# zpelgrims/zoic

Measured on AMD Instinct MI355X. Metric: camera rays/sec (Mrays/s), 4K x 16spp Kolb lens trace; ray-dir RMSE vs CPU ref, higher is better.
Workload: dtype f32

## Files before the change

### zoic_amd/csrc/device_search.hpp

```cpp
#pragma once
#include <hip/hip_runtime.h>

#include "optics.hpp"
#include "tables.hpp"

namespace zoic {

__device__ __forceinline__ int chunk_count_le(const float *chunk, float v)
{
    const float4 *p = reinterpret_cast<const float4 *>(chunk);
    const float4 a = p[0], b = p[1], c = p[2], d = p[3];
    int n = 0;
    n += !(v < a.x); n += !(v < a.y); n += !(v < a.z); n += !(v < a.w);
    n += !(v < b.x); n += !(v < b.y); n += !(v < b.z); n += !(v < b.w);
    n += !(v < c.x); n += !(v < c.y); n += !(v < c.z); n += !(v < c.w);
    n += !(v < d.x); n += !(v < d.y); n += !(v < d.z); n += !(v < d.w);
    return n;
}

__device__ __forceinline__ int pyramid_upper_bound(const float *const level[kBokehMaxLevels], const int32_t stride[kBokehMaxLevels],
                                                   const int32_t count[kBokehMaxLevels], int levels, int row, float v)
{
    int pos = 0;
#pragma unroll
// ... 9 lines not shown
__device__ __forceinline__ V2 bokeh_sample_device(const BokehTables &B, int x, int y, float uRow, float uCol)
{
    if (B.levels == 0)
        return bokeh_sample(B.cdfRow, B.rowIndices, B.cdfColumn, B.columnIndices, x, y, uRow, uCol);
    const int32_t zeroStride[kBokehMaxLevels] = {0, 0, 0};
    int r = pyramid_upper_bound(B.rowLevel, zeroStride, B.rowCount, B.levels, 0, uRow);
    if (r >= y) r = y - 1;
    const int row = B.rowIndices[r];
    int c = pyramid_upper_bound(B.colLevel, B.colStride, B.colCount, B.levels, row, uCol);
    if (c >= x) c = x - 1;
    const int start = row * x;
    const int col = B.columnIndices[start + c] - start;
    const float flippedRow = static_cast<float>(col - ((y - 1) / 2));
    const float flippedColumn = static_cast<float>(row - ((x - 1) / 2)) * -1.0f;
    return V2{(flippedRow / static_cast<float>(x)) * 2.0f, (flippedColumn / static_cast<float>(y)) * 2.0f};
}

__device__ __forceinline__ int cell_of(float u, int cellCount, bool &inRange)
{
    inRange = (u >= 0.0f) & (u < 1.0f);
    return inRange ? static_cast<int>(u * static_cast<float>(cellCount)) : 0;
}

__device__ __forceinline__ int cell_resolve(const uint4 rec, float u, bool inRange, bool &exceptional)
{
    const float a = __builtin_bit_cast(float, rec.x), b = __builtin_bit_cast(float, rec.y);
    const bool ge0 = !(u < a), ge1 = !(u < b);
    exceptional = ((rec.w >> 31) != 0u) | !inRange;
    const uint32_t pair = ge1 ? rec.w : rec.z;
    return static_cast<int>((ge0 & !ge1) ? (pair >> 16) : (pair & 0xffffu));
}

struct CellProbe { uint4 rec; int row; uint32_t cellIndex; };

__device__ __forceinline__ CellProbe bokeh_cells_issue(const BokehTables &B, const float *ldsRowCells, int y, float uRow, float uCol)
{
    bool inR, inC, excR;
    const int gr = cell_of(uRow, B.rowCellCount, inR);
    const int gc = cell_of(uCol, B.colCellCount, inC);
    int row = cell_resolve(reinterpret_cast<const uint4 *>(ldsRowCells)[gr], uRow, inR, excR);
    if (__ballot(excR) != 0ull) {
        if (excR) {
            const uint32_t bnd = B.rowBounds[gr];
            const int lo = inR ? static_cast<int>(bnd & 0xffffu) : 0, hi = inR ? static_cast<int>(bnd >> 16) : y;
            int r = lo + upper_bound_idx(B.cdfRow + lo, hi - lo, uRow);
            if (r >= y) r = y - 1;
            row = B.rowIndices[r];
        }
    }
    CellProbe p;
    p.row = row;
    p.cellIndex = static_cast<uint32_t>(row) * static_cast<uint32_t>(B.colCellCount) + static_cast<uint32_t>(gc);
    p.rec = reinterpret_cast<const uint4 *>(B.colCells)[p.cellIndex];
    return p;
}

template <bool EXACT_DIVIDE>
__device__ __forceinline__ V2 bokeh_cells_finish(const BokehTables &B, int x, int y, float uCol, const CellProbe &p)
{
    const bool inC = (uCol >= 0.0f) & (uCol < 1.0f);
    bool excC;
    const int row = p.row;
    int col = cell_resolve(p.rec, uCol, inC, excC);
    if (__ballot(excC) != 0ull) {
        if (excC) {
            const uint32_t bnd = B.colBounds[p.cellIndex];
            const int lo = inC ? static_cast<int>(bnd & 0xffffu) : 0, hi = inC ? static_cast<int>(bnd >> 16) : x;
            const int start = row * x;
            int c = lo + upper_bound_idx(B.cdfColumn + start + lo, hi - lo, uCol);
            if (c >= x) c = x - 1;
            col = B.columnIndices[start + c] - start;
        }
    }
    const float flippedRow = static_cast<float>(col - ((y - 1) / 2));
    const float flippedColumn = static_cast<float>(row - ((x - 1) / 2)) * -1.0f;
    if constexpr (EXACT_DIVIDE)
        return V2{(flippedRow / static_cast<float>(x)) * 2.0f, (flippedColumn / static_cast<float>(y)) * 2.0f};
    else
        return V2{flippedRow * (2.0f * __builtin_amdgcn_rcpf(static_cast<float>(x))),
                  flippedColumn * (2.0f * __builtin_amdgcn_rcpf(static_cast<float>(y)))};
}

template <bool EXACT_DIVIDE>
__device__ __forceinline__ V2 bokeh_sample_cells(const BokehTables &B, const float *ldsRowCells, int x, int y, float uRow, float uCol)
{
    return bokeh_cells_finish<EXACT_DIVIDE>(B, x, y, uCol, bokeh_cells_issue(B, ldsRowCells, y, uRow, uCol));
}

// ... 2 lines not shown
```

### zoic_amd/csrc/kolb_pool_body.hpp

```cpp
#pragma once
#include <hip/hip_runtime.h>

#include <cstdio>
#include <cstdlib>

#include "kolb_device.hpp"
#include "work_cursor.hpp"

#pragma STDC FP_CONTRACT OFF

#ifndef ZOIC_TWO_LEVEL_SEARCH
#define ZOIC_TWO_LEVEL_SEARCH 3
#endif
constexpr int kTwoLevelDraws = ZOIC_TWO_LEVEL_SEARCH;

namespace zoic {

struct KolbKernelArgs {
    KolbTable T; BokehTables B; const float4 *samples; const uint4 *rngStates; uint64_t rayBase; uint32_t n; RayRecord *out;
    DeviceCounters *counters; unsigned int *workCursor; uint32_t ldsWords, chunkRays, chunksPerPart, minSearching;
    uint32_t *redoList; unsigned int *redoCount;
    unsigned int *clearCursor;
};
template <class V, size_t OFFSET>
__device__ __forceinline__ V kernarg_field()
{
    typedef const char __attribute__((address_space(4))) *KernargBytes;
    KernargBytes base = (KernargBytes)__builtin_amdgcn_kernarg_segment_ptr();
    asm volatile("" : "+s"(base));
    return *(const V __attribute__((address_space(4))) *)(base + OFFSET);
}
#define ZOIC_KARG(field) kernarg_field<decltype(KolbKernelArgs::field), offsetof(KolbKernelArgs, field)>()

constexpr uint32_t kRetryDeadBit = 0x40000000u;

struct RaySetup { float o0x, o0y, maxScale, translation, sn, cs; uint32_t flags; bool dead, lutEdge; uint32_t rminq; };
template <bool STRICT, bool RMIN = false>
__device__ __forceinline__ RaySetup setup_ray(const KolbTable &T, const float2 *lutLds, float sx, float sy)
{
    RaySetup r;
    r.o0x = sx * T.halfSensor;
    r.o0y = sy * T.halfSensor;
    r.maxScale = 0.0f; r.translation = 0.0f; r.sn = 0.0f; r.cs = 1.0f; r.flags = 0u; r.dead = false; r.lutEdge = false; r.rminq = 0u;
    if (T.useLUT) {
        float dist;
// ... 75 lines not shown
    if (states) { const uint4 r = states[idx]; rng = Rng{r.x, r.y, r.z, r.w}; }
    else rng = rng_for_ray(T.seed, rayBase + idx);
    const DeadRayEnd e = dead_ray_end<STRICT>(T, B, bokehLds, rs, rng);
    store_ray_record(out, idx, e.o.x * -1.0f, e.o.y * -1.0f, e.o.z * -1.0f, e.d.x * -1.0f, e.d.y * -1.0f, e.d.z * -1.0f, e.w,
                     1u | (e.tries << 1) | ((rs.flags & 1u) << 6));
    return e.nanDraw;
}

#ifndef ZOIC_SEARCH_DRAWS
#define ZOIC_SEARCH_DRAWS 2
#endif
constexpr uint32_t kPoolEntries = 128;
constexpr uint32_t kPoolWaveWords = kPoolEntries * 12u;
constexpr uint32_t kPoolListWords = 128;
constexpr uint32_t kPoolTriesShift = 8, kPoolDeadBit = 1u << 13, kPoolRetryDeadBit = 1u << 14;

#ifndef ZOIC_POOL_ATTR_FAST
#define ZOIC_POOL_ATTR_FAST __attribute__((amdgpu_waves_per_eu(5, 8)))
#endif
#ifndef ZOIC_POOL_ATTR_STRICT
#define ZOIC_POOL_ATTR_STRICT __attribute__((amdgpu_waves_per_eu(4, 4)))
#endif

__device__ __forceinline__ uint32_t mask_rank(unsigned long long m)
{
    return __builtin_amdgcn_mbcnt_hi(static_cast<uint32_t>(m >> 32), __builtin_amdgcn_mbcnt_lo(static_cast<uint32_t>(m), 0u));
}
__device__ __forceinline__ bool mask_bit(unsigned long long m, uint32_t lane) { return ((m >> lane) & 1ull) != 0ull; }

constexpr uint32_t kShortList = 1u << 17;
template <bool STRICT, int NS, bool GUARD, bool DEAD, bool IMAGE, bool TWO = false>
__device__ __forceinline__ void kolb_pool_body(const KolbTable &T, const BokehTables &B, const float4 *__restrict__ samples,
                                               uint32_t n, RayRecord *__restrict__ out, uint32_t ldsWords, uint32_t minSearching)
{
    static_assert(!(GUARD && STRICT), "GUARD is a FAST mode");
    static_assert(!TWO || (DEAD && !IMAGE && kTwoLevelDraws > 0), "the two-level search belongs to the DEAD kernels of the disk sampler");
    constexpr bool DEFER = GUARD || DEAD;
    constexpr bool PROBE = IMAGE && !STRICT;
    constexpr uint32_t kOut = static_cast<uint32_t>(kMaxTries) + 1u;
    const uint32_t lane = threadIdx.x & 63u, wave = threadIdx.x >> 6;
    if (blockIdx.x == 0) {
        unsigned int *next = ZOIC_KARG(clearCursor);
        for (uint32_t i = threadIdx.x; i < kCursorBlockWords; i += kRefillBlock) next[i] = 0u;
    }
    if (threadIdx.x < kLutEntries) {
        zoicDynLds[2 * threadIdx.x] = T.lutMaxScale[threadIdx.x];
        zoicDynLds[2 * threadIdx.x + 1] = T.lutCentroidX[threadIdx.x];
    }
    const float *bokehLds = nullptr;
    if (IMAGE || ldsWords > 0) {
        for (uint32_t i = threadIdx.x; i < ldsWords; i += kRefillBlock) zoicDynLds[kLutLdsWords + i] = __builtin_bit_cast(float, B.rowCells[i]);
        bokehLds = zoicDynLds + kLutLdsWords;
    }
    __syncthreads();
    const float2 *lutLds = reinterpret_cast<const float2 *>(zoicDynLds);
    float4 *pool0 = reinterpret_cast<float4 *>(zoicDynLds + kLutLdsWords + ldsWords + wave * kPoolWaveWords);
    uint4 *pool2 = reinterpret_cast<uint4 *>(pool0 + kPoolEntries);
    float4 *pool1 = reinterpret_cast<float4 *>(pool2 + kPoolEntries);
    uint32_t *lists = reinterpret_cast<uint32_t *>(zoicDynLds + kLutLdsWords + ldsWords + kWavesPerBlock * kPoolWaveWords) +
                      wave * ((GUARD ? kPoolListWords : 0u) + (DEAD ? kPoolListWords : 0u));
    uint32_t *unsureLds = lists;
    uint32_t *deadLds = lists + (GUARD ? kPoolListWords : 0u);
    uint32_t poolCnt = 0, unsureCnt = 0, deadCnt = 0;

    const auto sample_lens = [&](float u, float v) {
        if constexpr (IMAGE) return bokeh_sample_cells<STRICT>(B, bokehLds, T.bokehW, T.bokehH, u, v);
        else return lens_sample<STRICT>(T, B, nullptr, u, v);
    };

    uint32_t next = 0, end = 0, part = blockIdx.x % kCursorParts, partsTried = 0;
    float4 s1 = make_float4(0.f, 0.f, 0.f, 0.f), s2 = s1;
    uint32_t base1 = 0, base2 = 0, cnt1 = 0, cnt2 = 0;
    bool have1 = false, have2 = false;
    CellProbe probe{make_uint4(0u, 0u, 0u, 0u), 0, 0u};
    const auto request_batch = [&]() {
        have2 = false;
        if (next >= end) {
            if (!claim_chunk(ZOIC_KARG(workCursor), lane, part, partsTried, ZOIC_KARG(chunkRays), ZOIC_KARG(chunksPerPart), n, next, end)) return;
        }
        base2 = next;
        cnt2 = (end - next < 64u) ? end - next : 64u;
        const uint32_t wi = (lane < cnt2) ? next + lane : next;
        s2 = samples[wi];
        next += cnt2;
        have2 = true;
    };
    const auto advance_batches = [&]() {
        s1 = s2; base1 = base2; cnt1 = cnt2; have1 = have2;
        if constexpr (PROBE) { if (have1) probe = bokeh_cells_issue(B, bokehLds, T.bokehH, s1.z, s1.w); }
        if (have1) request_batch();
    };
    request_batch();
    advance_batches();

    uint32_t succ = 0, vign = 0, tir = 0;
    uint32_t tirAcc = 0;

    constexpr bool memoryPhasesFirst = IMAGE;
    for (;;) {
        const bool drain = !have1;
        const bool fromPool = poolCnt >= 64u || (drain && poolCnt != 0u);
        if (!fromPool && drain) break;
        if (memoryPhasesFirst) __builtin_amdgcn_s_setprio(1);
        FastSurfaceTable fsurf = nullptr;
        if constexpr (GUARD) fsurf = launder_table(kernarg_fast_surfaces());
        else if constexpr (!STRICT) fsurf = kernarg_fast_surfaces();
        (void)fsurf;

        bool active, dead, unsure = false;
        uint32_t idx, tries, lutMiss;
        float o0x, o0y, maxScale, translation, sn, cs;
        uint32_t rminq = 0u;
        (void)rminq;
        Rng rng{1, 2, 3, 4};
        V3 o, d{0.0f, 0.0f, 1.0f};
        bool cand = false, finiteSample = true, searching;
        bool toFinish = false;
        const auto clears_rear = [&](const V3 &oo, const V3 &dd, bool &near0) {
            if constexpr (STRICT) {
                near0 = false;
                bool inRange;
                bool p = interface0_clear_strict_lean(T, oo, dd, inRange);
                if (__builtin_expect(!inRange, 0)) p = interface0_clear_strict(T, oo, dd);
                return p;
            }
            else return interface0_clear_fast<GUARD>(load_surface<false>(fsurf, 0), oo, dd, near0);
        };
        if (!fromPool) {
            active = lane < cnt1;
            idx = base1 + lane;
            const RaySetup rs = setup_ray<STRICT, TWO>(T, lutLds, s1.x, s1.y);
            o0x = rs.o0x; o0y = rs.o0y; maxScale = rs.maxScale; translation = rs.translation; sn = rs.sn; cs = rs.cs;
            lutMiss = rs.flags; dead = rs.dead; rminq = rs.rminq;
            if constexpr (GUARD) unsure = active && T.useLUT && rs.lutEdge;
            tries = 0;
            o = V3{o0x, o0y, T.originShift};
            searching = GUARD ? (active && !unsure) : active;
            const float u = s1.z, v = s1.w;
            V2 lens;
            const bool anyDead = __ballot(dead) != 0ull;
            bool plainSample = true;
            if (anyDead) plainSample = (u >= 0.0f) & (u < 1.0f) & (v >= 0.0f) & (v < 1.0f) & !((u == 0.5f) & (v == 0.5f));
            if constexpr (PROBE) lens = bokeh_cells_finish<STRICT>(B, T.bokehW, T.bokehH, v, probe);
            else {
                lens = V2{0.0f, 0.0f};
                if (__ballot(active && !(dead && plainSample)) != 0ull) lens = sample_lens(u, v);
            }
            if (anyDead) {
                if (dead && plainSample) lens = V2{0.0f, 0.0f};
                finiteSample = (fabsf(lens.x) <= 3.0e38f) && (fabsf(lens.y) <= 3.0e38f);
            }
            if (!T.useLUT) {
                d = V3{(lens.x * T.rearAperture) - o.x, (lens.y * T.rearAperture) - o.y, T.dirZ};
            } else {
                lens.x *= maxScale; lens.y *= maxScale;
                lens.x += translation;
                const float rx = lens.x * cs - lens.y * sn, ry = lens.x * sn + lens.y * cs;
                d = V3{rx - o.x, ry - o.y, T.dirZ};
            }
            bool near0 = false;
            bool pass0 = true;
            if (anyDead) pass0 = clears_rear(o, d, near0);
            if (searching) {
                if (GUARD && near0) { unsure = true; searching = false; }
                else if (pass0) { cand = true; searching = false; }
                else {
                    if (dead && finiteSample) { tries = kOut; searching = false; }
                    else if (DEAD && (lutMiss & kRetryDeadBit) != 0u) { toFinish = true; searching = false; }
                }
            }
        } else {
            const uint32_t cnt = poolCnt < 64u ? poolCnt : 64u;
            poolCnt -= cnt;
            active = lane < cnt;
            const uint32_t slot = poolCnt + (active ? lane : 0u);
            const float4 e0 = pool0[slot];
            const uint4 e2 = pool2[slot];
            const uint32_t packed = __builtin_bit_cast(uint32_t, e0.w);
            idx = __builtin_bit_cast(uint32_t, e0.x); o0x = e0.y; o0y = e0.z;
            const float4 e1 = pool1[slot];
            maxScale = e1.x; translation = e1.y; sn = e1.z; cs = e1.w;
            rng = Rng{e2.x, e2.y, e2.z, e2.w};
            tries = (packed >> kPoolTriesShift) & 31u;
            dead = (packed & kPoolDeadBit) != 0u;
            lutMiss = (packed & 0x7fu) | ((packed & kPoolRetryDeadBit) ? kRetryDeadBit : 0u);
            if constexpr (TWO) rminq = (packed >> 16) & 0xffu;
            o = V3{o0x, o0y, T.originShift};
            searching = active;
        }

        if (fromPool)
        for (;;) {
            const uint32_t looking = static_cast<uint32_t>(__popcll(__ballot(searching)));
            if (looking < (drain ? 1u : minSearching)) break;
            if (searching) {
                if (tries == 0) {
                    const uint4 *states = ZOIC_KARG(rngStates);
                    if (states) { const uint4 r = states[idx]; rng = Rng{r.x, r.y, r.z, r.w}; }
                    else rng = rng_for_ray(kernarg_field<uint32_t, offsetof(KolbKernelArgs, T) + offsetof(KolbTable, seed)>(), ZOIC_KARG(rayBase) + idx);
                }
                if constexpr (IMAGE && ZOIC_SEARCH_DRAWS > 1) {
                    constexpr int kDraws = ZOIC_SEARCH_DRAWS;
                    Rng after[kDraws];
                    float vCol[kDraws];
                    CellProbe probes[kDraws];
                    Rng r = rng;
#pragma unroll
                    for (int j = 0; j < kDraws; ++j) {
                        const float uj = rng_unit(xor128(r));
                        vCol[j] = rng_unit(xor128(r));
                        after[j] = r;
                        probes[j] = bokeh_cells_issue(B, bokehLds, T.bokehH, uj, vCol[j]);
                    }
                    bool open = true;
#pragma unroll
                    for (int j = 0; j < kDraws; ++j) {
                        if (open) {
                            ++tries; rng = after[j];
                            d = retry_direction(T, bokeh_cells_finish<STRICT>(B, T.bokehW, T.bokehH, vCol[j], probes[j]), o0x, o0y, maxScale, translation, sn, cs);
                            bool near0;
                            const bool pass0 = clears_rear(o, d, near0);
                            if (GUARD && near0) { unsure = true; searching = false; open = false; }
                            else if (pass0) { cand = true; searching = false; open = false; }
// ... 1 lines not shown
                        }
                    }
                } else {
                if constexpr (TWO) {  } else
                {
                const float u = rng_unit(xor128(rng));
                const float v = rng_unit(xor128(rng));
                ++tries;
                d = retry_direction(T, sample_lens(u, v), o0x, o0y, maxScale, translation, sn, cs);
                bool near0;
                const bool pass0 = clears_rear(o, d, near0);
                if (GUARD && near0) { unsure = true; searching = false; }
                else if (pass0) { cand = true; searching = false; }
                else if (tries > static_cast<uint32_t>(kMaxTries)) searching = false;
                }
                }
            }
            if constexpr (TWO) {
                bool pending = false;
                float pu = 0.0f, pv = 0.0f;
                const float rminf = static_cast<float>(rminq) * (1.0f / 256.0f);
#pragma unroll
                for (int k = 0; k < kTwoLevelDraws; ++k) {
                    if (k > 0 && __ballot(searching && !pending) == 0ull) break;
                    if (searching && !pending) {
                        pu = rng_unit(xor128(rng));
                        pv = rng_unit(xor128(rng));
                        ++tries;
                        const float rho = fmaxf(fabsf(ffma(2.0f, pu, -1.0f)), fabsf(ffma(2.0f, pv, -1.0f)));
                        const bool hopeless = (rho < rminf) & (rho > 0.0f);
                        pending = !hopeless | (tries > static_cast<uint32_t>(kMaxTries));
                    }
                }
                if (searching && pending) {
                    d = retry_direction(T, sample_lens(pu, pv), o0x, o0y, maxScale, translation, sn, cs);
                    bool near0;
                    const bool pass0 = clears_rear(o, d, near0);
                    if (GUARD && near0) { unsure = true; searching = false; }
                    else if (pass0) { cand = true; searching = false; }
                    else if (tries > static_cast<uint32_t>(kMaxTries)) searching = false;
                }
            }
        }

        if (!fromPool) advance_batches();

        bool ok = false;
        const V3 oStart = o, dStart = d;
        const bool firstTry = tries == 0;
        const unsigned long long candMask = __ballot(cand);
        if (candMask != 0ull) {
            if (memoryPhasesFirst) __builtin_amdgcn_s_setprio(0); else __builtin_amdgcn_s_setprio(3);
            uint32_t tirTry = 0;
            if constexpr (NS > 0) {
                if constexpr (STRICT) {
                    bool oor = false;
                    ok = trace_lens_strict_pred<NS>(T, o, d, tirTry, cand, oor);
                    if (__builtin_expect(__ballot(cand && oor) != 0ull, 0)) {
                        if (cand && oor) { o = oStart; d = dStart; tirTry = 0; ok = trace_lens_strict(T, o, d, tirTry); }
                    }
                } else {
                    unsigned long long tirMask, unsureMask;
                    const unsigned long long alive = trace_lens_fast_pred<NS, GUARD>(fsurf, o, d, candMask, tirMask, unsureMask);
                    ok = mask_bit(alive, lane);
                    tirTry = mask_bit(tirMask, lane) ? 1u : 0u;
                    if constexpr (GUARD) unsure |= mask_bit(unsureMask, lane);
                }
            } else if (cand) {
                if constexpr (STRICT) ok = trace_lens_strict(T, o, d, tirTry);
                else if constexpr (GUARD) { bool u2 = false; ok = trace_lens_fast_rolled(T, o, d, tirTry, &u2); unsure |= u2; }
                else ok = trace_lens_fast_rolled(T, o, d, tirTry);
            }
            const bool shortcut = cand && !ok && firstTry && dead && finiteSample && !(GUARD && unsure);
            if constexpr (DEFER) {
                if (!unsure) lutMiss += (tirTry << 1) + (shortcut ? (tirTry * kOut) << 1 : 0u);
            } else {
                tir += static_cast<uint32_t>(__popcll(__ballot(tirTry != 0u))) + kOut * static_cast<uint32_t>(__popcll(__ballot(shortcut && tirTry != 0u)));
            }
            if (shortcut) tries = kOut;
            else if (DEAD && cand && !ok && firstTry && (lutMiss & kRetryDeadBit) != 0u) toFinish = true;
            if constexpr (NS > 0) {
                if (cand && !ok && tries > static_cast<uint32_t>(kMaxTries) && !(GUARD && unsure)) {
                    uint32_t ignored = 0;
                    o = oStart; d = dStart;
                    if constexpr (STRICT) (void)trace_lens_strict(T, o, d, ignored);
                    else (void)trace_lens_fast_rolled(T, o, d, ignored);
                }
            }
        }
        if (!memoryPhasesFirst) __builtin_amdgcn_s_setprio(0);
        if (!cand) { o = oStart; d = dStart; }

        const bool dropU = GUARD && active && unsure;
        const bool dropF = DEAD && active && toFinish && !dropU;
        const bool finished = active && !searching && !toFinish && (ok || tries > static_cast<uint32_t>(kMaxTries)) && !dropU;
        if constexpr (DEFER) {
            if (finished || dropF) tirAcc += (lutMiss & ~kRetryDeadBit) >> 1;
        }
        {
            const uint32_t nv = static_cast<uint32_t>(__popcll(__ballot(finished && tries > static_cast<uint32_t>(kMaxTries))));
            vign += nv;
            succ += static_cast<uint32_t>(__popcll(__ballot(finished))) - nv;
        }
        {
            float w = (tries > static_cast<uint32_t>(kMaxTries)) ? 0.0f : 1.0f;
            if (T.exposureOn) w *= T.exposureMul;
            const uint32_t flags = (tries > 0 ? 1u : 0u) | (tries << 1) | ((lutMiss & 1u) << 6);
            constexpr bool kTransposed = IMAGE && !STRICT;
            if (kTransposed && !fromPool) {
                float4 *stA = pool0 + 64, *stB = reinterpret_cast<float4 *>(pool1) + 64;
                stA[lane] = make_float4(o.x * -1.0f, o.y * -1.0f, o.z * -1.0f, d.x * -1.0f);
                stB[lane] = make_float4(d.y * -1.0f, d.z * -1.0f, w, __builtin_bit_cast(float, flags));
                __builtin_amdgcn_wave_barrier();
                const unsigned long long fin = __ballot(finished);
                const float4 *half = (lane & 1u) ? stB : stA;
                float4 *dst = reinterpret_cast<float4 *>(out + (idx - lane));
                const float4 p0 = half[lane >> 1], p1 = half[32u + (lane >> 1)];
                if ((fin >> (lane >> 1)) & 1ull) dst[lane] = p0;
                if ((fin >> (32u + (lane >> 1))) & 1ull) dst[64u + lane] = p1;
                __builtin_amdgcn_wave_barrier();
            } else
            if (finished) {
                store_ray_record(out, idx, o.x * -1.0f, o.y * -1.0f, o.z * -1.0f, d.x * -1.0f, d.y * -1.0f, d.z * -1.0f, w, flags);
            }
        }
        if constexpr (GUARD) {
            const unsigned long long m = __ballot(dropU);
            if (m != 0ull) {
                if (dropU) unsureLds[unsureCnt + mask_rank(m)] = idx;
                unsureCnt += static_cast<uint32_t>(__popcll(m));
            }
        }
        if constexpr (DEAD) {
            const unsigned long long m = __ballot(dropF);
            if (m != 0ull) {
                if (dropF) deadLds[deadCnt + mask_rank(m)] = idx;
                deadCnt += static_cast<uint32_t>(__popcll(m));
            }
        }
        {
            const bool keep = active && !finished && !dropU && !dropF;
            const unsigned long long m = __ballot(keep);
            if (m != 0ull) {
                if (keep) {
                    const uint32_t slot = poolCnt + mask_rank(m);
                    uint32_t packed = (lutMiss & 0x7fu) | (tries << kPoolTriesShift) | (dead ? kPoolDeadBit : 0u) |
                                      ((lutMiss & kRetryDeadBit) ? kPoolRetryDeadBit : 0u);
                    if constexpr (TWO) packed |= rminq << 16;
                    pool0[slot] = make_float4(__builtin_bit_cast(float, idx), o0x, o0y, __builtin_bit_cast(float, packed));
                    pool1[slot] = make_float4(maxScale, translation, sn, cs);
                }
                if (__ballot(keep && tries != 0u) != 0ull) { if (keep) pool2[poolCnt + mask_rank(m)] = make_uint4(rng.x, rng.y, rng.z, rng.w); }
                poolCnt += static_cast<uint32_t>(__popcll(m));
            }
        }
        if constexpr (GUARD) {
            if (unsureCnt >= 64u) {
                uint32_t at = 0;
                if (lane == 0) at = atomicAdd(ZOIC_KARG(redoCount), unsureCnt);
                at = __builtin_amdgcn_readfirstlane(at);
                uint32_t *list = ZOIC_KARG(redoList);
                for (uint32_t j = lane; j < unsureCnt; j += 64u) list[at + j] = unsureLds[j];
                unsureCnt = 0;
            }
        }
        if constexpr (DEAD) {
            while (deadCnt >= 64u) {
                deadCnt -= 64u;
                const bool nanDraw = finish_dead_ray<STRICT>(T, B, lutLds, bokehLds, samples, ZOIC_KARG(rngStates), ZOIC_KARG(rayBase), out, deadLds[deadCnt + lane]);
                const uint32_t ns = static_cast<uint32_t>(__popcll(__ballot(nanDraw)));
                succ += ns; vign += 64u - ns;
            }
        }
    }

    if constexpr (GUARD) {
        if (unsureCnt != 0u) {
            uint32_t at = 0;
            if (lane == 0) at = atomicAdd(ZOIC_KARG(redoCount), unsureCnt);
            at = __builtin_amdgcn_readfirstlane(at);
            uint32_t *list = ZOIC_KARG(redoList);
            for (uint32_t j = lane; j < unsureCnt; j += 64u) list[at + j] = unsureLds[j];
        }
    }
    if constexpr (DEAD) {
        if (deadCnt != 0u) {
            const bool mine = lane < deadCnt;
            bool nanDraw = false;
            if (mine) nanDraw = finish_dead_ray<STRICT>(T, B, lutLds, bokehLds, samples, ZOIC_KARG(rngStates), ZOIC_KARG(rayBase), out, deadLds[lane]);
            const uint32_t ns = static_cast<uint32_t>(__popcll(__ballot(mine && nanDraw)));
            succ += ns; vign += deadCnt - ns;
        }
    }
    if constexpr (DEFER) {
        uint32_t t = tirAcc;
        for (int off = 32; off > 0; off >>= 1) t += __shfl_xor(t, off, 64);
        tir += static_cast<uint32_t>(__builtin_amdgcn_readfirstlane(static_cast<int>(t)));
    }
    DeviceCounters *counters = counter_set(ZOIC_KARG(counters));
    if (counters) {
        if (lane == 0) {
            if (succ) atomicAdd(&counters->succes, static_cast<unsigned long long>(succ));
            if (vign) atomicAdd(&counters->vignetted, static_cast<unsigned long long>(vign));
            if (tir) atomicAdd(&counters->tir, static_cast<unsigned long long>(tir));
        }
    }
}

#define ZOIC_POOL_PARAMS const KolbTable T, const BokehTables B, const float4 *__restrict__ samples, const uint4 *__restrict__ rngStates, \
        uint64_t rayBase, uint32_t n, RayRecord *__restrict__ out, DeviceCounters *counters, unsigned int *__restrict__ workCursor,        \
        uint32_t ldsWords, uint32_t chunkRays, uint32_t chunksPerPart, uint32_t minSearching, uint32_t *__restrict__ redoList,             \
        unsigned int *__restrict__ redoCount, unsigned int *__restrict__ clearCursor
#define ZOIC_POOL_KERNEL(NAME_, ATTR_, STRICT_, GUARD_)                                                                        \
    template <int NS, bool DEAD, bool IMAGE, bool TWO = false>                                                               \
    __global__ __launch_bounds__(kRefillBlock) ATTR_ void NAME_(ZOIC_POOL_PARAMS)                                             \
    {                                                                                                                        \
        kolb_pool_body<STRICT_, NS, GUARD_, DEAD, IMAGE, TWO>(T, B, samples, n, out, ldsWords, minSearching);                 \
    }
ZOIC_POOL_KERNEL(kolb_pool_strict_kernel, ZOIC_POOL_ATTR_STRICT, true, false)
ZOIC_POOL_KERNEL(kolb_pool_fast_kernel, ZOIC_POOL_ATTR_FAST, false, false)
ZOIC_POOL_KERNEL(kolb_pool_guard_kernel, ZOIC_POOL_ATTR_FAST, false, true)
#undef ZOIC_POOL_KERNEL
#undef ZOIC_POOL_PARAMS

int launch_kolb_listed(const KolbTable &table, const BokehTables &bokeh, const float4 *d_samples, const uint4 *d_rng, uint64_t rayBase, uint32_t m,
                       RayRecord *out, DeviceCounters *d_counters, unsigned int *d_redoCursor, uint32_t *d_redoList, unsigned int *d_redoCount,
                       unsigned grid, void *stream);

template <bool DEAD, bool IMAGE, bool TWO = false>
int launch_kolb_pool_impl(const KolbTable &table, const BokehTables &bokeh, const float *d_samples, const uint32_t *d_rng,
                          uint64_t rayBase, uint64_t n, RayRecord *out, DeviceCounters *d_counters, unsigned int *d_cursorPair, unsigned *parity,
                          int mode, uint32_t *d_scratch, void *stream)
{
    hipStream_t st = static_cast<hipStream_t>(stream);
    if (mode == 1 && !d_scratch) return static_cast<int>(hipErrorInvalidValue);
    constexpr uint64_t kMaxPerLaunch = 1ull << 31;
    uint32_t *d_redoList = d_scratch;
    for (uint64_t done = 0; done < n; done += kMaxPerLaunch) {
        const uint64_t m = (n - done < kMaxPerLaunch) ? (n - done) : kMaxPerLaunch;
        hipError_t e = hipSuccess;
        unsigned int *d_workCursor = d_cursorPair + (*parity & 1u) * kCursorBlockWords;
        unsigned int *d_clearCursor = d_cursorPair + ((*parity & 1u) ^ 1u) * kCursorBlockWords;
        *parity ^= 1u;
        const unsigned grid = persistent_grid(m, kWavesPerBlock);
        const WorkGrain grain = work_grain(m, mode == 0 ? 256u : 512u);
        const uint32_t chunkRays = grain.chunkRays, chunksPerPart = grain.chunksPerPart;
        RayRecord *o = out + done;
        const float4 *sp = reinterpret_cast<const float4 *>(d_samples) + done;
        const uint4 *rp = d_rng ? reinterpret_cast<const uint4 *>(d_rng) + done : nullptr;
        const uint32_t ldsWords = IMAGE ? static_cast<uint32_t>(bokeh.ldsWords) : 0u;
        const auto lds_bytes = [&](bool guard) {
            return static_cast<size_t>(ldsWords + kLutLdsWords + kWavesPerBlock * (kPoolWaveWords + (guard ? kPoolListWords : 0u) + (DEAD ? kPoolListWords : 0u))) * sizeof(float);
        };
        unsigned int *redoCount = d_workCursor + kRedoCountOffset, *redoCursor = d_workCursor + kRedoCursorOffset;
#define ZOIC_LAUNCH_POOL(KERNEL_, NS_, CURSOR_, GUARD_)                                                                          \
    hipLaunchKernelGGL((KERNEL_<NS_, DEAD, IMAGE, TWO>), dim3(grid), dim3(kRefillBlock), lds_bytes(GUARD_), st, table, bokeh, sp, rp, rayBase + done, \
                       static_cast<uint32_t>(m), o, d_counters, CURSOR_, ldsWords, chunkRays, chunksPerPart, kMinSearching, d_redoList, redoCount, d_clearCursor)
#define ZOIC_LAUNCH_POOL_BY_COUNT(KERNEL_, CURSOR_, GUARD_)                                                                      \
    switch (table.lensCount) {                     \
    case 7: ZOIC_LAUNCH_POOL(KERNEL_, 7, CURSOR_, GUARD_); break;                                                               \
    case 8: ZOIC_LAUNCH_POOL(KERNEL_, 8, CURSOR_, GUARD_); break;                                                               \
    case 9: ZOIC_LAUNCH_POOL(KERNEL_, 9, CURSOR_, GUARD_); break;                                                               \
    case 10: ZOIC_LAUNCH_POOL(KERNEL_, 10, CURSOR_, GUARD_); break;                                                             \
    case 11: ZOIC_LAUNCH_POOL(KERNEL_, 11, CURSOR_, GUARD_); break;                                                             \
    case 12: ZOIC_LAUNCH_POOL(KERNEL_, 12, CURSOR_, GUARD_); break;                                                             \
    default: ZOIC_LAUNCH_POOL(KERNEL_, 0, CURSOR_, GUARD_); break;                                                              \
    }
        if (mode == 0) { ZOIC_LAUNCH_POOL_BY_COUNT(kolb_pool_strict_kernel, d_workCursor, false) }
        else if (mode == 2) { ZOIC_LAUNCH_POOL_BY_COUNT(kolb_pool_fast_kernel, d_workCursor, false) }
        else {
            ZOIC_LAUNCH_POOL_BY_COUNT(kolb_pool_guard_kernel, d_workCursor, true)
            e = hipGetLastError();
            if (e != hipSuccess) return static_cast<int>(e);
            e = static_cast<hipError_t>(launch_kolb_listed(table, bokeh, sp, rp, rayBase + done, static_cast<uint32_t>(m), o, d_counters, redoCursor,
                                                           d_redoList, redoCount, grid, stream));
        }
#undef ZOIC_LAUNCH_POOL_BY_COUNT
#undef ZOIC_LAUNCH_POOL
        e = hipGetLastError();
        if (e != hipSuccess) return static_cast<int>(e);
// ... 11 lines not shown
```

### zoic_amd/csrc/optics.hpp

```cpp
#pragma once
#include <cmath>
#include <cstdint>

#include "tables.hpp"

#if defined(__HIP_DEVICE_COMPILE__)
#include "exact_math.hpp"
#define ZOIC_SQRT_RN(x) ::zoic::sqrt_rn(x)
#define ZOIC_RCP_RN(x) ::zoic::rcp_rn(x)
#else
#define ZOIC_SQRT_RN(x) sqrtf(x)
#define ZOIC_RCP_RN(x) (1.0f / (x))
#endif

#pragma STDC FP_CONTRACT OFF

namespace zoic {

struct V3 { float x, y, z; };
struct V2 { float x, y; };

constexpr float kPi = 3.14159265358979323846f;
constexpr float kTwoPi = kPi * 2;
constexpr float kPiOver2 = 1.57079632679489661923f;
// ... 9 lines not shown
}

struct Rng { uint32_t x, y, z, w; };

ZOIC_HD void rng_seed_reference(Rng &r) { r = Rng{123456789u, 362436069u, 521288629u, 88675123u}; }

ZOIC_HD uint32_t xor128(Rng &r)
{
    uint32_t t = r.x ^ (r.x << 11);
    r.x = r.y; r.y = r.z; r.z = r.w;
    r.w = r.w ^ (r.w >> 19) ^ t ^ (t >> 8);
    return r.w;
}

ZOIC_HD float rng_unit(uint32_t u) { return static_cast<float>(u) * kInv2p32; }

ZOIC_HD uint32_t pcg_hash(uint32_t v)
{
    uint32_t state = v * 747796405u + 2891336453u;
    uint32_t word = ((state >> ((state >> 28u) + 4u)) ^ state) * 277803737u;
    return (word >> 22u) ^ word;
}

ZOIC_HD Rng rng_for_ray(uint32_t seed, uint64_t gid)
{
    uint32_t lo = static_cast<uint32_t>(gid), hi = static_cast<uint32_t>(gid >> 32);
    uint32_t k = pcg_hash(seed ^ pcg_hash(hi + 0x9E3779B9u));
    Rng r;
    r.x = pcg_hash(k ^ (lo * 4u + 0u));
    r.y = pcg_hash(k ^ (lo * 4u + 1u) ^ 0x85EBCA6Bu);
    r.z = pcg_hash(k ^ (lo * 4u + 2u) ^ 0xC2B2AE35u);
    r.w = pcg_hash(k ^ (lo * 4u + 3u) ^ 0x27D4EB2Fu) | 1u;
    return r;
}

ZOIC_HD float wrap_to_pi(float x)
{
    float v = x + kPi;
    if (v >= kTwoPi) v = v - kTwoPi;
    return v - kPi;
}

ZOIC_HD float parabola_sin(float x)
{
    const float B = 4.0f / kPi;
    const float C = -4.0f / (kPi * kPi);
    float y = B * x + C * x * fabsf(x);
    const float P = 0.225f;
    return P * (y * fabsf(y) - y) + y;
}

ZOIC_HD float fast_sin(float x) { return parabola_sin(wrap_to_pi(x)); }

ZOIC_HD float fast_cos(float x)
{
    x = static_cast<float>(static_cast<double>(x) + static_cast<double>(kPi) * 0.5);
// ... 127 lines not shown
```

Baseline: 44250.

## Move per-lane predicates to wave-uniform ballot masks and precompute RNG seed key

Replaces per-lane boolean state (active, searching, cand, unsure, finished, keep) in the pool kernel with 64-bit wave masks held in scalar registers, using inverse_ballot to drive predication. The goal is to cut VGPR pressure and repeated ballot instructions. The per-ray RNG seeding is hoisted out of the search loop into the pool load, and the high-word hash is computed once on the host and passed as a new seedKey kernel argument. Some address computations are also rewritten as byte offsets to allow scalar base plus lane offset addressing. The restructuring is broad, so scalar register pressure or predication behaviour may shift in ways that are hard to anticipate.

```diff
diff --git a/zoic_amd/csrc/device_search.hpp b/zoic_amd/csrc/device_search.hpp
--- a/zoic_amd/csrc/device_search.hpp
+++ b/zoic_amd/csrc/device_search.hpp
@@ -55,11 +55,11 @@
     return inRange ? static_cast<int>(u * static_cast<float>(cellCount)) : 0;
 }
 
-__device__ __forceinline__ int cell_resolve(const uint4 rec, float u, bool inRange, bool &exceptional)
+__device__ __forceinline__ int cell_resolve(const uint4 rec, float u, unsigned long long &exceptional)
 {
     const float a = __builtin_bit_cast(float, rec.x), b = __builtin_bit_cast(float, rec.y);
     const bool ge0 = !(u < a), ge1 = !(u < b);
-    exceptional = ((rec.w >> 31) != 0u) | !inRange;
+    exceptional = __builtin_amdgcn_ballot_w64(static_cast<int32_t>(rec.w) < 0) | __builtin_amdgcn_ballot_w64(!(u >= 0.0f)) | __builtin_amdgcn_ballot_w64(!(u < 1.0f));
     const uint32_t pair = ge1 ? rec.w : rec.z;
     return static_cast<int>((ge0 & !ge1) ? (pair >> 16) : (pair & 0xffffu));
 }
@@ -68,12 +68,13 @@
 
 __device__ __forceinline__ CellProbe bokeh_cells_issue(const BokehTables &B, const float *ldsRowCells, int y, float uRow, float uCol)
 {
-    bool inR, inC, excR;
+    bool inR, inC;
+    unsigned long long excR;
     const int gr = cell_of(uRow, B.rowCellCount, inR);
     const int gc = cell_of(uCol, B.colCellCount, inC);
-    int row = cell_resolve(reinterpret_cast<const uint4 *>(ldsRowCells)[gr], uRow, inR, excR);
-    if (__ballot(excR) != 0ull) {
-        if (excR) {
+    int row = cell_resolve(reinterpret_cast<const uint4 *>(ldsRowCells)[gr], uRow, excR);
+    if (excR != 0ull) {
+        if (__builtin_amdgcn_inverse_ballot_w64(excR)) {
             const uint32_t bnd = B.rowBounds[gr];
             const int lo = inR ? static_cast<int>(bnd & 0xffffu) : 0, hi = inR ? static_cast<int>(bnd >> 16) : y;
             int r = lo + upper_bound_idx(B.cdfRow + lo, hi - lo, uRow);
@@ -84,7 +85,7 @@
     CellProbe p;
     p.row = row;
     p.cellIndex = static_cast<uint32_t>(row) * static_cast<uint32_t>(B.colCellCount) + static_cast<uint32_t>(gc);
-    p.rec = reinterpret_cast<const uint4 *>(B.colCells)[p.cellIndex];
+    p.rec = *reinterpret_cast<const uint4 *>(reinterpret_cast<const char *>(B.colCells) + p.cellIndex * 16u);
     return p;
 }
 
@@ -92,11 +93,11 @@
 __device__ __forceinline__ V2 bokeh_cells_finish(const BokehTables &B, int x, int y, float uCol, const CellProbe &p)
 {
     const bool inC = (uCol >= 0.0f) & (uCol < 1.0f);
-    bool excC;
+    unsigned long long excC;
     const int row = p.row;
-    int col = cell_resolve(p.rec, uCol, inC, excC);
-    if (__ballot(excC) != 0ull) {
-        if (excC) {
+    int col = cell_resolve(p.rec, uCol, excC);
+    if (excC != 0ull) {
+        if (__builtin_amdgcn_inverse_ballot_w64(excC)) {
             const uint32_t bnd = B.colBounds[p.cellIndex];
             const int lo = inC ? static_cast<int>(bnd & 0xffffu) : 0, hi = inC ? static_cast<int>(bnd >> 16) : x;
             const int start = row * x;
diff --git a/zoic_amd/csrc/kolb_pool_body.hpp b/zoic_amd/csrc/kolb_pool_body.hpp
--- a/zoic_amd/csrc/kolb_pool_body.hpp
+++ b/zoic_amd/csrc/kolb_pool_body.hpp
@@ -21,6 +21,7 @@
     DeviceCounters *counters; unsigned int *workCursor; uint32_t ldsWords, chunkRays, chunksPerPart, minSearching;
     uint32_t *redoList; unsigned int *redoCount;
     unsigned int *clearCursor;
+    uint32_t seedKey;
 };
 template <class V, size_t OFFSET>
 __device__ __forceinline__ V kernarg_field()
@@ -142,9 +143,16 @@
 #define ZOIC_POOL_ATTR_STRICT __attribute__((amdgpu_waves_per_eu(4, 4)))
 #endif
 
+__device__ __forceinline__ unsigned long long wave_ballot(bool p) { return __builtin_amdgcn_ballot_w64(p); }
 __device__ __forceinline__ uint32_t mask_rank(unsigned long long m)
 {
     return __builtin_amdgcn_mbcnt_hi(static_cast<uint32_t>(m >> 32), __builtin_amdgcn_mbcnt_lo(static_cast<uint32_t>(m), 0u));
+}
+__device__ __forceinline__ unsigned long long double_bits(uint32_t m)
+{
+    unsigned long long r;
+    asm("s_bitreplicate_b64_b32 %0, %1" : "=s"(r) : "s"(m));
+    return r;
 }
 __device__ __forceinline__ bool mask_bit(unsigned long long m, uint32_t lane) { return ((m >> lane) & 1ull) != 0ull; }
 
@@ -191,19 +199,19 @@
     uint32_t next = 0, end = 0, part = blockIdx.x % kCursorParts, partsTried = 0;
     float4 s1 = make_float4(0.f, 0.f, 0.f, 0.f), s2 = s1;
     uint32_t base1 = 0, base2 = 0, cnt1 = 0, cnt2 = 0;
-    bool have1 = false, have2 = false;
+    uint32_t have1 = 0u, have2 = 0u;
     CellProbe probe{make_uint4(0u, 0u, 0u, 0u), 0, 0u};
     const auto request_batch = [&]() {
-        have2 = false;
+        have2 = 0u;
         if (next >= end) {
             if (!claim_chunk(ZOIC_KARG(workCursor), lane, part, partsTried, ZOIC_KARG(chunkRays), ZOIC_KARG(chunksPerPart), n, next, end)) return;
         }
         base2 = next;
         cnt2 = (end - next < 64u) ? end - next : 64u;
-        const uint32_t wi = (lane < cnt2) ? next + lane : next;
-        s2 = samples[wi];
+        const uint32_t wl = (lane < cnt2) ? lane : 0u;
+        s2 = *reinterpret_cast<const float4 *>(reinterpret_cast<const char *>(samples + next) + wl * 16u);
         next += cnt2;
-        have2 = true;
+        have2 = 1u;
     };
     const auto advance_batches = [&]() {
         s1 = s2; base1 = base2; cnt1 = cnt2; have1 = have2;
@@ -218,24 +226,30 @@
 
     constexpr bool memoryPhasesFirst = IMAGE;
     for (;;) {
-        const bool drain = !have1;
+        const bool drain = have1 == 0u;
         const bool fromPool = poolCnt >= 64u || (drain && poolCnt != 0u);
         if (!fromPool && drain) break;
         if (memoryPhasesFirst) __builtin_amdgcn_s_setprio(1);
         FastSurfaceTable fsurf = nullptr;
-        if constexpr (GUARD) fsurf = launder_table(kernarg_fast_surfaces());
+        if constexpr (GUARD) {
+            typedef const char __attribute__((address_space(4))) *KernargBytes;
+            KernargBytes kb = (KernargBytes)__builtin_amdgcn_kernarg_segment_ptr();
+            asm volatile("" : "+s"(kb));
+            fsurf = (FastSurfaceTable)(kb + offsetof(KolbTable, fsurf));
+        }
         else if constexpr (!STRICT) fsurf = kernarg_fast_surfaces();
         (void)fsurf;
 
-        bool active, dead, unsure = false;
+        bool active, dead;
         uint32_t idx, tries, lutMiss;
         float o0x, o0y, maxScale, translation, sn, cs;
         uint32_t rminq = 0u;
         (void)rminq;
         Rng rng{1, 2, 3, 4};
         V3 o, d{0.0f, 0.0f, 1.0f};
-        bool cand = false, finiteSample = true, searching;
-        bool toFinish = false;
+        bool finiteSample = true;
+        uint32_t passBase = 0u;
+        unsigned long long activeM, searchingM, candMask = 0ull, unsureM = 0ull, toFinishM = 0ull, deadM, finiteM = ~0ull;
         const auto clears_rear = [&](const V3 &oo, const V3 &dd, bool &near0) {
             if constexpr (STRICT) {
                 near0 = false;
@@ -247,28 +261,32 @@
             else return interface0_clear_fast<GUARD>(load_surface<false>(fsurf, 0), oo, dd, near0);
         };
         if (!fromPool) {
+            activeM = cnt1 >= 64u ? ~0ull : (1ull << cnt1) - 1ull;
+            passBase = base1;
             active = lane < cnt1;
             idx = base1 + lane;
             const RaySetup rs = setup_ray<STRICT, TWO>(T, lutLds, s1.x, s1.y);
             o0x = rs.o0x; o0y = rs.o0y; maxScale = rs.maxScale; translation = rs.translation; sn = rs.sn; cs = rs.cs;
             lutMiss = rs.flags; dead = rs.dead; rminq = rs.rminq;
-            if constexpr (GUARD) unsure = active && T.useLUT && rs.lutEdge;
+            if constexpr (GUARD) { if (T.useLUT) unsureM = activeM & wave_ballot(rs.lutEdge); }
             tries = 0;
             o = V3{o0x, o0y, T.originShift};
-            searching = GUARD ? (active && !unsure) : active;
+            searchingM = activeM & ~unsureM;
             const float u = s1.z, v = s1.w;
             V2 lens;
-            const bool anyDead = __ballot(dead) != 0ull;
+            deadM = wave_ballot(dead);
+            const bool anyDead = deadM != 0ull;
             bool plainSample = true;
             if (anyDead) plainSample = (u >= 0.0f) & (u < 1.0f) & (v >= 0.0f) & (v < 1.0f) & !((u == 0.5f) & (v == 0.5f));
             if constexpr (PROBE) lens = bokeh_cells_finish<STRICT>(B, T.bokehW, T.bokehH, v, probe);
             else {
                 lens = V2{0.0f, 0.0f};
-                if (__ballot(active && !(dead && plainSample)) != 0ull) lens = sample_lens(u, v);
+                if (wave_ballot(active && !(dead && plainSample)) != 0ull) lens = sample_lens(u, v);
             }
             if (anyDead) {
                 if (dead && plainSample) lens = V2{0.0f, 0.0f};
                 finiteSample = (fabsf(lens.x) <= 3.0e38f) && (fabsf(lens.y) <= 3.0e38f);
+                finiteM = wave_ballot(finiteSample);
             }
             if (!T.useLUT) {
                 d = V3{(lens.x * T.rearAperture) - o.x, (lens.y * T.rearAperture) - o.y, T.dirZ};
@@ -278,20 +296,29 @@
                 const float rx = lens.x * cs - lens.y * sn, ry = lens.x * sn + lens.y * cs;
                 d = V3{rx - o.x, ry - o.y, T.dirZ};
             }
-            bool near0 = false;
-            bool pass0 = true;
-            if (anyDead) pass0 = clears_rear(o, d, near0);
-            if (searching) {
-                if (GUARD && near0) { unsure = true; searching = false; }
-                else if (pass0) { cand = true; searching = false; }
-                else {
-                    if (dead && finiteSample) { tries = kOut; searching = false; }
-                    else if (DEAD && (lutMiss & kRetryDeadBit) != 0u) { toFinish = true; searching = false; }
+            if (!anyDead) { candMask = searchingM; searchingM = 0ull; }
+            else {
+                bool near0 = false;
+                const bool pass0 = clears_rear(o, d, near0);
+                if constexpr (GUARD) {
+                    const unsigned long long nearM = searchingM & wave_ballot(near0);
+                    unsureM |= nearM; searchingM &= ~nearM;
+                }
+                candMask = searchingM & wave_ballot(pass0);
+                searchingM &= ~candMask;
+                const unsigned long long outNowM = searchingM & deadM & finiteM;
+                if (__builtin_amdgcn_inverse_ballot_w64(outNowM)) tries = kOut;
+                searchingM &= ~outNowM;
+                if constexpr (DEAD) {
+                    toFinishM = searchingM & wave_ballot((lutMiss & kRetryDeadBit) != 0u);
+                    searchingM &= ~toFinishM;
                 }
             }
         } else {
             const uint32_t cnt = poolCnt < 64u ? poolCnt : 64u;
             poolCnt -= cnt;
+            activeM = cnt >= 64u ? ~0ull : (1ull << cnt) - 1ull;
+            searchingM = activeM;
             active = lane < cnt;
             const uint32_t slot = poolCnt + (active ? lane : 0u);
             const float4 e0 = pool0[slot];
@@ -303,22 +330,30 @@
             rng = Rng{e2.x, e2.y, e2.z, e2.w};
             tries = (packed >> kPoolTriesShift) & 31u;
             dead = (packed & kPoolDeadBit) != 0u;
+            deadM = wave_ballot(dead);
             lutMiss = (packed & 0x7fu) | ((packed & kPoolRetryDeadBit) ? kRetryDeadBit : 0u);
             if constexpr (TWO) rminq = (packed >> 16) & 0xffu;
             o = V3{o0x, o0y, T.originShift};
-            searching = active;
-        }
-
-        if (fromPool)
+            if (tries == 0u) {
+                const uint4 *states = ZOIC_KARG(rngStates);
+                if (states) { const uint4 r = states[idx]; rng = Rng{r.x, r.y, r.z, r.w}; }
+                else {
+                    const uint64_t rayBase = ZOIC_KARG(rayBase);
+                    const uint32_t baseLo = static_cast<uint32_t>(rayBase), lo = baseLo + idx;
+                    uint32_t key = ZOIC_KARG(seedKey);
+                    if (__builtin_expect(lo < baseLo, 0))
+                        key = rng_key(kernarg_field<uint32_t, offsetof(KolbKernelArgs, T) + offsetof(KolbTable, seed)>(), static_cast<uint32_t>(rayBase >> 32) + 1u);
+                    rng = rng_from_key(key, lo);
+                }
+            }
+        }
+
+        if (fromPool) {
+        bool searching = active, cand = false, unsure = false;
         for (;;) {
-            const uint32_t looking = static_cast<uint32_t>(__popcll(__ballot(searching)));
+            const uint32_t looking = static_cast<uint32_t>(__popcll(wave_ballot(searching)));
             if (looking < (drain ? 1u : minSearching)) break;
             if (searching) {
-                if (tries == 0) {
-                    const uint4 *states = ZOIC_KARG(rngStates);
-                    if (states) { const uint4 r = states[idx]; rng = Rng{r.x, r.y, r.z, r.w}; }
-                    else rng = rng_for_ray(kernarg_field<uint32_t, offsetof(KolbKernelArgs, T) + offsetof(KolbTable, seed)>(), ZOIC_KARG(rayBase) + idx);
-                }
                 if constexpr (IMAGE && ZOIC_SEARCH_DRAWS > 1) {
                     constexpr int kDraws = ZOIC_SEARCH_DRAWS;
                     Rng after[kDraws];
@@ -366,7 +401,7 @@
                 const float rminf = static_cast<float>(rminq) * (1.0f / 256.0f);
 #pragma unroll
                 for (int k = 0; k < kTwoLevelDraws; ++k) {
-                    if (k > 0 && __ballot(searching && !pending) == 0ull) break;
+                    if (k > 0 && wave_ballot(searching && !pending) == 0ull) break;
                     if (searching && !pending) {
                         pu = rng_unit(xor128(rng));
                         pv = rng_unit(xor128(rng));
@@ -387,67 +422,90 @@
             }
         }
 
+        candMask = wave_ballot(cand); searchingM = wave_ballot(searching);
+        if constexpr (GUARD) unsureM = wave_ballot(unsure);
+        }
+
         if (!fromPool) advance_batches();
 
-        bool ok = false;
+        const unsigned long long firstTryM = wave_ballot(tries == 0u);
+        unsigned long long outM = wave_ballot(tries > static_cast<uint32_t>(kMaxTries));
+        unsigned long long deadFirstM = firstTryM & deadM & finiteM;
+        asm volatile("" : "+s"(deadFirstM));
+
+        unsigned long long okM = 0ull;
         const V3 oStart = o, dStart = d;
-        const bool firstTry = tries == 0;
-        const unsigned long long candMask = __ballot(cand);
         if (candMask != 0ull) {
             if (memoryPhasesFirst) __builtin_amdgcn_s_setprio(0); else __builtin_amdgcn_s_setprio(3);
-            uint32_t tirTry = 0;
-            if constexpr (NS > 0) {
-                if constexpr (STRICT) {
+            unsigned long long tirM;
+            if constexpr (NS > 0 && !STRICT) {
+                unsigned long long unsureMask;
+                okM = trace_lens_fast_pred<NS, GUARD>(fsurf, o, d, candMask, tirM, unsureMask);
+                if constexpr (GUARD) unsureM |= unsureMask;
+            } else {
+                const bool cand = __builtin_amdgcn_inverse_ballot_w64(candMask);
+                bool ok = false, unsure = false;
+                uint32_t tirTry = 0;
+                if constexpr (NS > 0) {
                     bool oor = false;
                     ok = trace_lens_strict_pred<NS>(T, o, d, tirTry, cand, oor);
-                    if (__builtin_expect(__ballot(cand && oor) != 0ull, 0)) {
+                    if (__builtin_expect(wave_ballot(cand && oor) != 0ull, 0)) {
                         if (cand && oor) { o = oStart; d = dStart; tirTry = 0; ok = trace_lens_strict(T, o, d, tirTry); }
                     }
-                } else {
-                    unsigned long long tirMask, unsureMask;
-                    const unsigned long long alive = trace_lens_fast_pred<NS, GUARD>(fsurf, o, d, candMask, tirMask, unsureMask);
-                    ok = mask_bit(alive, lane);
-                    tirTry = mask_bit(tirMask, lane) ? 1u : 0u;
-                    if constexpr (GUARD) unsure |= mask_bit(unsureMask, lane);
-                }
-            } else if (cand) {
-                if constexpr (STRICT) ok = trace_lens_strict(T, o, d, tirTry);
-                else if constexpr (GUARD) { bool u2 = false; ok = trace_lens_fast_rolled(T, o, d, tirTry, &u2); unsure |= u2; }
-                else ok = trace_lens_fast_rolled(T, o, d, tirTry);
-            }
-            const bool shortcut = cand && !ok && firstTry && dead && finiteSample && !(GUARD && unsure);
+                } else if (cand) {
+                    if constexpr (STRICT) ok = trace_lens_strict(T, o, d, tirTry);
+                    else if constexpr (GUARD) { bool u2 = false; ok = trace_lens_fast_rolled(T, o, d, tirTry, &u2); unsure |= u2; }
+                    else ok = trace_lens_fast_rolled(T, o, d, tirTry);
+                }
+                okM = wave_ballot(ok);
+                tirM = wave_ballot(tirTry != 0u);
+                if constexpr (GUARD) unsureM |= wave_ballot(unsure);
+            }
+            const unsigned long long shortcutM = candMask & ~okM & deadFirstM & ~unsureM;
             if constexpr (DEFER) {
-                if (!unsure) lutMiss += (tirTry << 1) + (shortcut ? (tirTry * kOut) << 1 : 0u);
+                const unsigned long long bumpM = tirM & ~unsureM;
+                if (bumpM != 0ull) {
+                    if (__builtin_amdgcn_inverse_ballot_w64(bumpM)) lutMiss += 1u << 1;
+                    if (__builtin_amdgcn_inverse_ballot_w64(bumpM & shortcutM)) lutMiss += kOut << 1;
+                }
             } else {
-                tir += static_cast<uint32_t>(__popcll(__ballot(tirTry != 0u))) + kOut * static_cast<uint32_t>(__popcll(__ballot(shortcut && tirTry != 0u)));
-            }
-            if (shortcut) tries = kOut;
-            else if (DEAD && cand && !ok && firstTry && (lutMiss & kRetryDeadBit) != 0u) toFinish = true;
+                tir += static_cast<uint32_t>(__popcll(tirM)) + kOut * static_cast<uint32_t>(__popcll(shortcutM & tirM));
+            }
+            if (shortcutM != 0ull) {
+                if (__builtin_amdgcn_inverse_ballot_w64(shortcutM)) tries = kOut;
+                outM |= shortcutM;
+            }
+            if constexpr (DEAD) toFinishM |= candMask & ~okM & firstTryM & ~shortcutM & wave_ballot((lutMiss & kRetryDeadBit) != 0u);
             if constexpr (NS > 0) {
-                if (cand && !ok && tries > static_cast<uint32_t>(kMaxTries) && !(GUARD && unsure)) {
-                    uint32_t ignored = 0;
-                    o = oStart; d = dStart;
-                    if constexpr (STRICT) (void)trace_lens_strict(T, o, d, ignored);
-                    else (void)trace_lens_fast_rolled(T, o, d, ignored);
+                const unsigned long long againM = candMask & ~okM & outM & ~unsureM;
+                if (againM != 0ull) {
+                    if (__builtin_amdgcn_inverse_ballot_w64(againM)) {
+                        uint32_t ignored = 0;
+                        o = oStart; d = dStart;
+                        if constexpr (STRICT) (void)trace_lens_strict(T, o, d, ignored);
+                        else (void)trace_lens_fast_rolled(T, o, d, ignored);
+                    }
                 }
             }
         }
         if (!memoryPhasesFirst) __builtin_amdgcn_s_setprio(0);
-        if (!cand) { o = oStart; d = dStart; }
-
-        const bool dropU = GUARD && active && unsure;
-        const bool dropF = DEAD && active && toFinish && !dropU;
-        const bool finished = active && !searching && !toFinish && (ok || tries > static_cast<uint32_t>(kMaxTries)) && !dropU;
+
+        const unsigned long long dropUM = GUARD ? activeM & unsureM : 0ull;
+        const unsigned long long dropFM = DEAD ? activeM & toFinishM & ~dropUM : 0ull;
+        const unsigned long long finishedM = activeM & ~searchingM & ~toFinishM & (okM | outM) & ~dropUM;
+        if ((finishedM & ~candMask) != 0ull) {
+            if (__builtin_amdgcn_inverse_ballot_w64(finishedM & ~candMask)) { o = oStart; d = dStart; }
+        }
         if constexpr (DEFER) {
-            if (finished || dropF) tirAcc += (lutMiss & ~kRetryDeadBit) >> 1;
+            if (__builtin_amdgcn_inverse_ballot_w64(finishedM | dropFM)) tirAcc += (lutMiss & ~kRetryDeadBit) >> 1;
         }
         {
-            const uint32_t nv = static_cast<uint32_t>(__popcll(__ballot(finished && tries > static_cast<uint32_t>(kMaxTries))));
+            const uint32_t nv = static_cast<uint32_t>(__popcll(finishedM & outM));
             vign += nv;
-            succ += static_cast<uint32_t>(__popcll(__ballot(finished))) - nv;
+            succ += static_cast<uint32_t>(__popcll(finishedM)) - nv;
         }
         {
-            float w = (tries > static_cast<uint32_t>(kMaxTries)) ? 0.0f : 1.0f;
+            float w = __builtin_amdgcn_inverse_ballot_w64(outM) ? 0.0f : 1.0f;
             if (T.exposureOn) w *= T.exposureMul;
             const uint32_t flags = (tries > 0 ? 1u : 0u) | (tries << 1) | ((lutMiss & 1u) << 6);
             constexpr bool kTransposed = IMAGE && !STRICT;
@@ -456,46 +514,43 @@
                 stA[lane] = make_float4(o.x * -1.0f, o.y * -1.0f, o.z * -1.0f, d.x * -1.0f);
                 stB[lane] = make_float4(d.y * -1.0f, d.z * -1.0f, w, __builtin_bit_cast(float, flags));
                 __builtin_amdgcn_wave_barrier();
-                const unsigned long long fin = __ballot(finished);
                 const float4 *half = (lane & 1u) ? stB : stA;
-                float4 *dst = reinterpret_cast<float4 *>(out + (idx - lane));
+                char *dst = reinterpret_cast<char *>(out + passBase);
                 const float4 p0 = half[lane >> 1], p1 = half[32u + (lane >> 1)];
-                if ((fin >> (lane >> 1)) & 1ull) dst[lane] = p0;
-                if ((fin >> (32u + (lane >> 1))) & 1ull) dst[64u + lane] = p1;
+                if (__builtin_amdgcn_inverse_ballot_w64(double_bits(static_cast<uint32_t>(finishedM)))) *reinterpret_cast<float4 *>(dst + lane * 16u) = p0;
+                if (__builtin_amdgcn_inverse_ballot_w64(double_bits(static_cast<uint32_t>(finishedM >> 32)))) *reinterpret_cast<float4 *>(dst + (1024u + lane * 16u)) = p1;
                 __builtin_amdgcn_wave_barrier();
             } else
-            if (finished) {
+            if (__builtin_amdgcn_inverse_ballot_w64(finishedM)) {
                 store_ray_record(out, idx, o.x * -1.0f, o.y * -1.0f, o.z * -1.0f, d.x * -1.0f, d.y * -1.0f, d.z * -1.0f, w, flags);
             }
         }
         if constexpr (GUARD) {
-            const unsigned long long m = __ballot(dropU);
-            if (m != 0ull) {
-                if (dropU) unsureLds[unsureCnt + mask_rank(m)] = idx;
-                unsureCnt += static_cast<uint32_t>(__popcll(m));
+            if (dropUM != 0ull) {
+                if (__builtin_amdgcn_inverse_ballot_w64(dropUM)) unsureLds[unsureCnt + mask_rank(dropUM)] = idx;
+                unsureCnt += static_cast<uint32_t>(__popcll(dropUM));
             }
         }
         if constexpr (DEAD) {
-            const unsigned long long m = __ballot(dropF);
-            if (m != 0ull) {
-                if (dropF) deadLds[deadCnt + mask_rank(m)] = idx;
-                deadCnt += static_cast<uint32_t>(__popcll(m));
+            if (dropFM != 0ull) {
+                if (__builtin_amdgcn_inverse_ballot_w64(dropFM)) deadLds[deadCnt + mask_rank(dropFM)] = idx;
+                deadCnt += static_cast<uint32_t>(__popcll(dropFM));
             }
         }
         {
-            const bool keep = active && !finished && !dropU && !dropF;
-            const unsigned long long m = __ballot(keep);
-            if (m != 0ull) {
-                if (keep) {
-                    const uint32_t slot = poolCnt + mask_rank(m);
-                    uint32_t packed = (lutMiss & 0x7fu) | (tries << kPoolTriesShift) | (dead ? kPoolDeadBit : 0u) |
+            const unsigned long long keepM = activeM & ~finishedM & ~dropUM & ~dropFM;
+            if (keepM != 0ull) {
+                const uint32_t slot = poolCnt + mask_rank(keepM);
+                if (__builtin_amdgcn_inverse_ballot_w64(keepM)) {
+                    uint32_t packed = (lutMiss & 0x7fu) | (tries << kPoolTriesShift) | (__builtin_amdgcn_inverse_ballot_w64(deadM) ? kPoolDeadBit : 0u) |
                                       ((lutMiss & kRetryDeadBit) ? kPoolRetryDeadBit : 0u);
                     if constexpr (TWO) packed |= rminq << 16;
                     pool0[slot] = make_float4(__builtin_bit_cast(float, idx), o0x, o0y, __builtin_bit_cast(float, packed));
                     pool1[slot] = make_float4(maxScale, translation, sn, cs);
                 }
-                if (__ballot(keep && tries != 0u) != 0ull) { if (keep) pool2[poolCnt + mask_rank(m)] = make_uint4(rng.x, rng.y, rng.z, rng.w); }
-                poolCnt += static_cast<uint32_t>(__popcll(m));
+                const unsigned long long drawnM = keepM & wave_ballot(tries != 0u);
+                if (drawnM != 0ull) { if (__builtin_amdgcn_inverse_ballot_w64(keepM)) pool2[slot] = make_uint4(rng.x, rng.y, rng.z, rng.w); }
+                poolCnt += static_cast<uint32_t>(__popcll(keepM));
             }
         }
         if constexpr (GUARD) {
@@ -512,7 +567,7 @@
             while (deadCnt >= 64u) {
                 deadCnt -= 64u;
                 const bool nanDraw = finish_dead_ray<STRICT>(T, B, lutLds, bokehLds, samples, ZOIC_KARG(rngStates), ZOIC_KARG(rayBase), out, deadLds[deadCnt + lane]);
-                const uint32_t ns = static_cast<uint32_t>(__popcll(__ballot(nanDraw)));
+                const uint32_t ns = static_cast<uint32_t>(__popcll(wave_ballot(nanDraw)));
                 succ += ns; vign += 64u - ns;
             }
         }
@@ -532,7 +587,7 @@
             const bool mine = lane < deadCnt;
             bool nanDraw = false;
             if (mine) nanDraw = finish_dead_ray<STRICT>(T, B, lutLds, bokehLds, samples, ZOIC_KARG(rngStates), ZOIC_KARG(rayBase), out, deadLds[lane]);
-            const uint32_t ns = static_cast<uint32_t>(__popcll(__ballot(mine && nanDraw)));
+            const uint32_t ns = static_cast<uint32_t>(__popcll(wave_ballot(mine && nanDraw)));
             succ += ns; vign += deadCnt - ns;
         }
     }
@@ -554,7 +609,7 @@
 #define ZOIC_POOL_PARAMS const KolbTable T, const BokehTables B, const float4 *__restrict__ samples, const uint4 *__restrict__ rngStates, \
         uint64_t rayBase, uint32_t n, RayRecord *__restrict__ out, DeviceCounters *counters, unsigned int *__restrict__ workCursor,        \
         uint32_t ldsWords, uint32_t chunkRays, uint32_t chunksPerPart, uint32_t minSearching, uint32_t *__restrict__ redoList,             \
-        unsigned int *__restrict__ redoCount, unsigned int *__restrict__ clearCursor
+        unsigned int *__restrict__ redoCount, unsigned int *__restrict__ clearCursor, uint32_t seedKey
 #define ZOIC_POOL_KERNEL(NAME_, ATTR_, STRICT_, GUARD_)                                                                        \
     template <int NS, bool DEAD, bool IMAGE, bool TWO = false>                                                               \
     __global__ __launch_bounds__(kRefillBlock) ATTR_ void NAME_(ZOIC_POOL_PARAMS)                                             \
@@ -592,6 +647,7 @@
         RayRecord *o = out + done;
         const float4 *sp = reinterpret_cast<const float4 *>(d_samples) + done;
         const uint4 *rp = d_rng ? reinterpret_cast<const uint4 *>(d_rng) + done : nullptr;
+        const uint32_t seedKey = rng_key(table.seed, static_cast<uint32_t>((rayBase + done) >> 32));
         const uint32_t ldsWords = IMAGE ? static_cast<uint32_t>(bokeh.ldsWords) : 0u;
         const auto lds_bytes = [&](bool guard) {
             return static_cast<size_t>(ldsWords + kLutLdsWords + kWavesPerBlock * (kPoolWaveWords + (guard ? kPoolListWords : 0u) + (DEAD ? kPoolListWords : 0u))) * sizeof(float);
@@ -599,7 +655,7 @@
         unsigned int *redoCount = d_workCursor + kRedoCountOffset, *redoCursor = d_workCursor + kRedoCursorOffset;
 #define ZOIC_LAUNCH_POOL(KERNEL_, NS_, CURSOR_, GUARD_)                                                                          \
     hipLaunchKernelGGL((KERNEL_<NS_, DEAD, IMAGE, TWO>), dim3(grid), dim3(kRefillBlock), lds_bytes(GUARD_), st, table, bokeh, sp, rp, rayBase + done, \
-                       static_cast<uint32_t>(m), o, d_counters, CURSOR_, ldsWords, chunkRays, chunksPerPart, kMinSearching, d_redoList, redoCount, d_clearCursor)
+                       static_cast<uint32_t>(m), o, d_counters, CURSOR_, ldsWords, chunkRays, chunksPerPart, kMinSearching, d_redoList, redoCount, d_clearCursor, seedKey)
 #define ZOIC_LAUNCH_POOL_BY_COUNT(KERNEL_, CURSOR_, GUARD_)                                                                      \
     switch (table.lensCount) {                     \
     case 7: ZOIC_LAUNCH_POOL(KERNEL_, 7, CURSOR_, GUARD_); break;                                                               \
diff --git a/zoic_amd/csrc/optics.hpp b/zoic_amd/csrc/optics.hpp
--- a/zoic_amd/csrc/optics.hpp
+++ b/zoic_amd/csrc/optics.hpp
@@ -55,16 +55,19 @@
     return (word >> 22u) ^ word;
 }
 
-ZOIC_HD Rng rng_for_ray(uint32_t seed, uint64_t gid)
-{
-    uint32_t lo = static_cast<uint32_t>(gid), hi = static_cast<uint32_t>(gid >> 32);
-    uint32_t k = pcg_hash(seed ^ pcg_hash(hi + 0x9E3779B9u));
+ZOIC_HD uint32_t rng_key(uint32_t seed, uint32_t hi) { return pcg_hash(seed ^ pcg_hash(hi + 0x9E3779B9u)); }
+ZOIC_HD Rng rng_from_key(uint32_t k, uint32_t lo)
+{
     Rng r;
     r.x = pcg_hash(k ^ (lo * 4u + 0u));
     r.y = pcg_hash(k ^ (lo * 4u + 1u) ^ 0x85EBCA6Bu);
     r.z = pcg_hash(k ^ (lo * 4u + 2u) ^ 0xC2B2AE35u);
     r.w = pcg_hash(k ^ (lo * 4u + 3u) ^ 0x27D4EB2Fu) | 1u;
     return r;
+}
+ZOIC_HD Rng rng_for_ray(uint32_t seed, uint64_t gid)
+{
+    return rng_from_key(rng_key(seed, static_cast<uint32_t>(gid >> 32)), static_cast<uint32_t>(gid));
 }
 
 ZOIC_HD float wrap_to_pi(float x)
```

Measured after the change: 47120 (median of 6 runs). 6.5% higher.
